# yharby/flac-raster

Hardware: AMD Instinct MI355X
Metric: raster MPixels/sec encoded at -c 5 + size ratio vs libFLAC, 1/2/4/8 GPU (higher is better)
Workload: dtype u16->i16 (int32 analysis, exact integer autocorrelation on i8 MFMA)

## Files before the change

### flac-raster_amd/csrc/fra_analyze_w.hip

```cpp
#include <type_traits>

#include "fra_device.h"

namespace fra {

namespace {

constexpr int kWChunks = kMaxBlock / kChunk;
constexpr int kWIters = kWChunks / 64;

struct WaveSmem {
  uint32_t sw[8 * kWChunks];
  double acf[3][9];
};
constexpr uint32_t kBufWords = 8 * kWChunks;

__device__ __forceinline__ int sdw(int t, int d) { return 8 * t + d; }
__device__ __forceinline__ int32_t wsample(const uint32_t* sw, int s) {
  const uint32_t v = sw[sdw(s >> 4, (s & 15) >> 1)];
  return (s & 1) ? hi16(v) : lo16(v);
}
__device__ __forceinline__ void wsync() {
  __builtin_amdgcn_wave_barrier();
  asm volatile("" ::: "memory");
}
constexpr int kWIterDw = 8 * 64;
constexpr int kWinW = 3;
__device__ __forceinline__ uint4 lds4(const uint32_t* p) { return *reinterpret_cast<const uint4*>(p); }
__device__ __forceinline__ void wread_d14(const uint32_t* sw, int lane, int j, uint32_t (&D)[14]) {
  const uint32_t* po = sw + 8 * lane + kWIterDw * j;
  const bool first = j == 0 && lane == 0;
  const uint32_t* pp = first ? po : po - 8;
  const uint4 p0 = lds4(pp), p1 = lds4(pp + 4), o0 = lds4(po), o1 = lds4(po + 4);
  D[0] = first ? 0u : p0.z; D[1] = first ? 0u : p0.w;
  D[2] = first ? 0u : p1.x; D[3] = first ? 0u : p1.y; D[4] = first ? 0u : p1.z; D[5] = first ? 0u : p1.w;
  D[6] = o0.x; D[7] = o0.y; D[8] = o0.z; D[9] = o0.w;
  D[10] = o1.x; D[11] = o1.y; D[12] = o1.z; D[13] = o1.w;
}
__device__ __forceinline__ void unpack28(const uint32_t (&D)[14], int32_t (&x)[28]) {
#pragma unroll
  for (int k = 0; k < 14; k++) {
    x[2 * k] = lo16(D[k]);
    x[2 * k + 1] = hi16(D[k]);
  }
}
__device__ __forceinline__ uint32_t group_sum32(uint32_t v, int ls) {
  if (ls > 0) v = up_add32<0>(v);
  if (ls > 1) v = up_add32<1>(v);
  if (ls > 2) v = up_add32<2>(v);
  if (ls > 3) v = up_add32<3>(v);
  if (ls > 4) v = up_add32<4>(v);
  if (ls > 5) v = up_add32<5>(v);
  return v;
}
__device__ __forceinline__ uint64_t group_sum64(uint64_t v, int ls) {
  if (ls > 0) v = up_add64<0>(v);
  if (ls > 1) v = up_add64<1>(v);
  if (ls > 2) v = up_add64<2>(v);
  if (ls > 3) v = up_add64<3>(v);
  if (ls > 4) v = up_add64<4>(v);
  if (ls > 5) v = up_add64<5>(v);
  return v;
}
__device__ __forceinline__ uint64_t group_sum_auto(uint64_t v, int ls) {
  if (__all(v < (1ull << (32 - ls)))) return group_sum32((uint32_t)v, ls);
  return group_sum64(v, ls);
}
__device__ __forceinline__ double rdlane_f64(double v, int l) {
  const uint64_t b = (uint64_t)__double_as_longlong(v);
  const uint32_t lo = (uint32_t)__builtin_amdgcn_readlane((int)(uint32_t)b, l);
  const uint32_t hi = (uint32_t)__builtin_amdgcn_readlane((int)(uint32_t)(b >> 32), l);
  return __longlong_as_double((long long)(((uint64_t)hi << 32) | lo));
}


__device__ __forceinline__ int32_t wround16(float x, float w) {
  return __float_as_int(__fadd_rn(__fmul_rn(x, w), 12582912.0f));
}

template <int MAXLAG>
__device__ inline int levinson_keep(const double (&ac)[MAXLAG + 1], int max_order, double& e, double (&lp)[MAXLAG],
                                    int lo) {
  double lpc[MAXLAG];
#pragma unroll
  for (int j = 0; j < MAXLAG; j++) { lpc[j] = 0.0; lp[j] = 0.0; }
  e = 0.0;
  double err = ac[0];
  int result = max_order;
  bool done = false;
#pragma unroll
  for (int i = 0; i < MAXLAG; i++) {
    if (!done && i < max_order) {
      double r = -ac[i + 1];
#pragma unroll
      for (int j = 0; j < i; j++) r = r - lpc[j] * ac[i - j];
      r = r / err;
      lpc[i] = r;
#pragma unroll
      for (int j = 0; j < (i >> 1); j++) {
        const double tmp = lpc[j];
        lpc[j] = lpc[j] + r * lpc[i - 1 - j];
        lpc[i - 1 - j] = lpc[i - 1 - j] + r * tmp;
      }
      if (i & 1) lpc[i >> 1] = lpc[i >> 1] + lpc[i >> 1] * r;
      err = err * (1.0 - r * r);
      const bool mine = lo == i + 1;
#pragma unroll
      for (int j = 0; j <= i; j++) lp[j] = mine ? -lpc[j] : lp[j];
      e = (mine || (i == 0 && lo == 0)) ? err : e;
      if (!(err > 0.0)) {
        result = (err == 0.0) ? i + 1 : i;
        done = true;
      }
    }
  }
  return result;
}

__device__ __forceinline__ void fixed_guess2_w(const uint32_t (&ps)[5], int P, int lane, int& g1, int& g2,
                                               uint64_t& t1, uint64_t& t2) {
  uint64_t T[5];
  bool small = true;
  uint32_t pv[5];
#pragma unroll
  for (int k = 0; k < 5; k++) {
    pv[k] = lane < (1 << P) ? ps[k] : 0u;
    small = small && pv[k] < (1u << 25);
  }
  if (__all(small)) {
#pragma unroll
    for (int k = 0; k < 5; k++) T[k] = wave_sum32(pv[k]);
  } else {
#pragma unroll
    for (int k = 0; k < 5; k++) {
      uint64_t v = pv[k];
      v = up_add64<0>(v); v = up_add64<1>(v); v = up_add64<2>(v);
      v = up_add64<3>(v); v = up_add64<4>(v); v = up_add64<5>(v);
      T[k] = ((uint64_t)(uint32_t)__builtin_amdgcn_readlane((int)(uint32_t)(v >> 32), 63) << 32) |
             (uint32_t)__builtin_amdgcn_readlane((int)(uint32_t)v, 63);
    }
  }
  int h1 = -1, h2 = -1;
  uint64_t b1 = 0, b2 = 0;
#pragma unroll
  for (int k = 0; k < 5; k++) {
    const bool lt1 = h1 < 0 || T[k] < b1;
    const bool lt2 = !lt1 && (h2 < 0 || T[k] < b2);
    b2 = lt1 ? b1 : (lt2 ? T[k] : b2);
    h2 = lt1 ? h1 : (lt2 ? k : h2);
    b1 = lt1 ? T[k] : b1;
    h1 = lt1 ? k : h1;
  }
  g1 = __builtin_amdgcn_readfirstlane(h1);
  g2 = __builtin_amdgcn_readfirstlane(h2);
  t1 = b1;
  t2 = b2;
}

#ifndef FRA_W_ARITH
#define FRA_W_ARITH 0
#endif
struct WNorm {
  double two_mn, range, rcp;
  uint32_t flip;
};
template <typename T>
__device__ __forceinline__ int32_t wnorm(uint32_t r, const WNorm& q) {
  const int32_t v = (int32_t)((r ^ q.flip) - q.flip);
  const double t = fma((double)v, 2.0, q.two_mn);
  const double q0 = t * q.rcp;
  const double rr = fma(-q0, q.range, t);
  double u = fma(rr, q.rcp, q0);
  u = u - 1.0;
  u = u * 32767.0;
  return (int32_t)u;
}
template <typename T>
__device__ __forceinline__ void wload_lut(const void* base, const WaveDev& wd, int c,
                                          const int32_t* lut, uint32_t* sw, int lane, uint32_t& orv, uint32_t& anv,
                                          bool stamp, const WNorm& wn) {
  constexpr int V = 8 / (int)sizeof(T);
  constexpr int NV = kMaxBlock / 64 / V;
  constexpr uint32_t step = 64 * V;
  using VT = VecT<T, V>;
  const uint32_t w = wd.width;
  const char* b0 = (const char*)((const T*)base + wd.off0 + (int64_t)c * wd.band_stride);
  const uint32_t rsb = wd.row_stride * (uint32_t)sizeof(T);
  const uint32_t qs = step / w, rs = step - qs * w, rstep = qs * rsb;
  uint32_t col = wd.col0 + (uint32_t)lane * V;
  uint32_t roff = 0;
  if (col >= w) {
    const uint32_t q = col / w;
    col -= q * w;
    roff = q * rsb;
  }
  VT x[NV];
#pragma unroll
  for (int kv = 0; kv < NV; kv++) {
    x[kv] = *(const VT*)(b0 + (roff + col * (uint32_t)sizeof(T)));
    col += rs;
    roff += rstep;
    if (col >= w) { col -= w; roff += rsb; }
  }
  if (stamp) FRA_WSTAMP_WAIT(11)
  uint32_t orp = 0, anp = 0xFFFFFFFFu;
#pragma unroll
  for (int kv = 0; kv < NV; kv++) {
    int32_t g[V];
    const bool arith = FRA_W_ARITH == 1 || (FRA_W_ARITH == 2 && (kv & 1));
    const uint2 xw = __builtin_bit_cast(uint2, x[kv]);
#pragma unroll
    for (int e = 0; e < V; e++) {
      constexpr int EB = 8 * (int)sizeof(T);
      const uint32_t wsrc = e < V / 2 ? xw.x : xw.y;
      const uint32_t raw = (wsrc >> (EB * (e % (V / 2)))) & ((1u << EB) - 1u);
      uint32_t off = raw << 2;
      asm("" : "+v"(off));
      g[e] = arith ? wnorm<T>(raw, wn) : *(const int32_t*)((const char*)lut + off);
    }
    const int i = (lane + 64 * kv) * V;
#pragma unroll
    for (int h = 0; h < V / 4; h++) {
      const int s = i + 4 * h;
      const uint32_t p0 = __builtin_amdgcn_perm((uint32_t)g[4 * h + 1], (uint32_t)g[4 * h], 0x05040100u);
      const uint32_t p1 = __builtin_amdgcn_perm((uint32_t)g[4 * h + 3], (uint32_t)g[4 * h + 2], 0x05040100u);
      *reinterpret_cast<uint2*>(&sw[sdw(s >> 4, (s & 15) >> 1)]) = make_uint2(p0, p1);
      orp |= p0 | p1;
      anp &= p0 & p1;
    }
  }
  orv |= (orp | (orp >> 16)) & 0xFFFFu;
  anv &= anp & (anp >> 16);
  if (stamp) FRA_WSTAMP_WAIT(12)
}

#define FRA_DOT4(a, b, c, d, q, c0, c1, c2, c3)                   \
  "v_dot2_i32_i16 %[p0], %[x" #a "], %[q" #q "], " c0 "\n\t"      \
  "v_dot2_i32_i16 %[p1], %[x" #b "], %[q" #q "], " c1 "\n\t"      \
  "v_dot2_i32_i16 %[p2], %[x" #c "], %[q" #q "], " c2 "\n\t"      \
  "v_dot2_i32_i16 %[p3], %[x" #d "], %[q" #q "], " c3 "\n\t"
#define FRA_DOT4_FIRST(a, b, c, d, q) FRA_DOT4(a, b, c, d, q, "0", "0", "0", "0")
#define FRA_DOT4_NEXT(a, b, c, d, q) FRA_DOT4(a, b, c, d, q, "%[p0]", "%[p1]", "%[p2]", "%[p3]")
#define FRA_SHR4                              \
  "v_ashrrev_i32 %[p0], %[sh], %[p0]\n\t"     \
  "v_ashrrev_i32 %[p1], %[sh], %[p1]\n\t"     \
  "v_ashrrev_i32 %[p2], %[sh], %[p2]\n\t"     \
  "v_ashrrev_i32 %[p3], %[sh], %[p3]"
#define FRA_P4_OUT [p0] "=&v"(p[0]), [p1] "=&v"(p[1]), [p2] "=&v"(p[2]), [p3] "=&v"(p[3])
template <int NP>
__device__ __forceinline__ void pred4_w(const uint32_t (&D)[14], int b, const fra_short2 (&Q)[NP], int sh,
                                        int32_t (&p)[4]) {
  static_assert(NP >= 1 && NP <= 4, "orders 1-8");
  uint32_t X[2 * NP + 2];
#pragma unroll
  for (int k = 0; k < 2 * NP + 2; k++) X[k] = pair_at(D, b - 2 * NP + k);
  if constexpr (NP == 1) {
    asm(FRA_DOT4_FIRST(0, 1, 2, 3, 0) FRA_SHR4
        : FRA_P4_OUT
        : [sh] "s"(sh), [q0] "s"(Q[0]), [x0] "v"(X[0]), [x1] "v"(X[1]), [x2] "v"(X[2]), [x3] "v"(X[3]));
  } else if constexpr (NP == 2) {
    asm(FRA_DOT4_FIRST(2, 3, 4, 5, 0) FRA_DOT4_NEXT(0, 1, 2, 3, 1) FRA_SHR4
        : FRA_P4_OUT
        : [sh] "s"(sh), [q0] "s"(Q[0]), [q1] "s"(Q[1]), [x0] "v"(X[0]), [x1] "v"(X[1]), [x2] "v"(X[2]), [x3] "v"(X[3]),
          [x4] "v"(X[4]), [x5] "v"(X[5]));
  } else if constexpr (NP == 3) {
    asm(FRA_DOT4_FIRST(4, 5, 6, 7, 0) FRA_DOT4_NEXT(2, 3, 4, 5, 1) FRA_DOT4_NEXT(0, 1, 2, 3, 2) FRA_SHR4
        : FRA_P4_OUT
        : [sh] "s"(sh), [q0] "s"(Q[0]), [q1] "s"(Q[1]), [q2] "s"(Q[2]), [x0] "v"(X[0]), [x1] "v"(X[1]), [x2] "v"(X[2]),
          [x3] "v"(X[3]), [x4] "v"(X[4]), [x5] "v"(X[5]), [x6] "v"(X[6]), [x7] "v"(X[7]));
  } else {
    asm(FRA_DOT4_FIRST(6, 7, 8, 9, 0) FRA_DOT4_NEXT(4, 5, 6, 7, 1) FRA_DOT4_NEXT(2, 3, 4, 5, 2)
        FRA_DOT4_NEXT(0, 1, 2, 3, 3) FRA_SHR4
        : FRA_P4_OUT
        : [sh] "s"(sh), [q0] "s"(Q[0]), [q1] "s"(Q[1]), [q2] "s"(Q[2]), [q3] "s"(Q[3]), [x0] "v"(X[0]), [x1] "v"(X[1]),
          [x2] "v"(X[2]), [x3] "v"(X[3]), [x4] "v"(X[4]), [x5] "v"(X[5]), [x6] "v"(X[6]), [x7] "v"(X[7]), [x8] "v"(X[8]),
          [x9] "v"(X[9]));
  }
}
#undef FRA_P4_OUT
#undef FRA_SHR4
#undef FRA_DOT4_NEXT
#undef FRA_DOT4_FIRST
#undef FRA_DOT4

template <int O>
__device__ __forceinline__ uint32_t lpc_abs16_w(const uint32_t (&D)[14], const int32_t* q, int sh, bool head) {
  constexpr int NP = (O + 1) / 2;
  fra_short2 Q[NP];
  q_pairs_rev<NP>(q, Q);
  uint32_t acc = 0;
#pragma unroll
  for (int jb = 0; jb < kChunk; jb += 4) {
    int32_t p[4];
    pred4_w<NP>(D, 12 + jb, Q, sh, p);
#pragma unroll
    for (int i = 0; i < 4; i++) {
      const int jj = jb + i;
      const int32_t r = sample_at(D, 12 + jj) - p[i];
      const uint32_t rb = (uint32_t)r ^ kBias;
      acc = sad_acc(rb, (jj < O && head) ? rb : kBias, acc);
    }
  }
  return acc;
}

template <int O, bool K17>
__device__ __forceinline__ uint32_t lpc_abs16_pk(const uint32_t (&D)[14], const int32_t* q, int sh, bool head,
                                                 uint32_t (&pk)[kChunk / 2], uint32_t& um, uint32_t& hb) {
  constexpr int NP = (O + 1) / 2;
  fra_short2 Q[NP];
  q_pairs_rev<NP>(q, Q);
  uint32_t su = 0, ss = 0;
  uint32_t u[kChunk];
  hb = 0;
#pragma unroll
  for (int jb = 0; jb < kChunk; jb += 4) {
    int32_t p[4];
    pred4_w<NP>(D, 12 + jb, Q, sh, p);
#pragma unroll
    for (int i = 0; i < 4; i++) {
      const int jj = jb + i;
      const int32_t r = sample_at(D, 12 + jj) - p[i];
      uint32_t sg = (uint32_t)(r >> 31);
      asm("" : "+v"(sg));
      const bool warm = jj < O && head;
      u[jj] = warm ? 0u : (((uint32_t)r << 1) ^ sg);
      su += u[jj];
      ss += warm ? 0u : sg;
      um |= u[jj];
    }
  }
  const uint32_t acc = su - ss;
#pragma unroll
  for (int p = 0; p < kChunk / 2; p++) pk[p] = __builtin_amdgcn_perm(u[2 * p + 1], u[2 * p], 0x05040100u);
  if (K17 && __any(um > 0xFFFFu)) {
#pragma unroll
    for (int jj = 0; jj < kChunk; jj++) hb |= (u[jj] >> 16) << jj;
  }
  return acc;
}

}


template <int MAXLAG, int PCAP, bool K17>
#ifndef FRA_W_WAVES
#define FRA_W_WAVES 4
#endif
#ifndef FRA_W_ACF_ITERS
#define FRA_W_ACF_ITERS 4
#endif
#ifndef FRA_W_VGPR_FLOOR
#define FRA_W_VGPR_FLOOR 1
#endif
#ifndef FRA_W_WAVES_MAX
#define FRA_W_WAVES_MAX 8
#endif
__global__ void __launch_bounds__(64) __attribute__((amdgpu_waves_per_eu(FRA_W_WAVES, FRA_W_WAVES_MAX)))
k_analyze_w(JobArgs a, int src) {
  static_assert(MAXLAG == 8 && PCAP >= 4 && PCAP <= 6, "levels 3-6");
  __shared__ WaveSmem S;
  uint32_t* const sw = S.sw;
  const int lane = (int)threadIdx.x;
#if FRA_W_VGPR_FLOOR
  asm volatile("" ::: "v103");
#endif
  FRA_WSTAMP(0)
#ifndef FRA_W_XCD
#define FRA_W_XCD 1
#endif
  int bx = (int)blockIdx.x;
  if (FRA_W_XCD) {
    const int nx = (int)gridDim.x, n8 = nx & ~7;
    const int lin = bx + (int)blockIdx.y * nx;
    if ((nx & 7) == 0 && bx < n8) bx = (lin & 7) * (n8 >> 3) + (bx >> 3);
  }
  const int g = a.frame_base + bx;
  const int c = (int)blockIdx.y;
  const WaveDev wd = a.wave[g];
  if (c >= wd.nch) return;
  FRA_WSTAMP_WAIT(10)
  if (wd.n != kMaxBlock) return;
  constexpr int n = kMaxBlock;
  const int bps = wd.bps;
  const LevelCfg cfg = level_cfg(a.level);
  SfDesc* d = &a.sf[(size_t)g * a.cmax + c];
  uint32_t* const slot = a.tmp + ((size_t)g * a.cmax + c) * a.tmp_stride;
#ifdef FRA_WSTOP
  if (lane == 0) {
    d->type = 1; d->order = 0; d->wasted = 0; d->sbps = (uint8_t)bps; d->cval = 0; d->porder = 0;
    d->method = 0; d->precision = 0; d->shift = 0; d->bits = 8u + (uint32_t)n * (uint32_t)bps;
  }
#endif

  uint32_t orv = 0, anv = 0xFFFFu;
  const void* const raster = a.raster;
  const int32_t* const lut = a.lut + (int64_t)wd.stream * a.lut_stride;
  WNorm wn{};
  if (FRA_W_ARITH) {
    const NormParams np = norm_params(a.streams[wd.stream], a.norm[wd.stream]);
    wn.two_mn = -2.0 * np.mn;
    wn.range = np.range;
    wn.rcp = np.rcp;
    wn.flip = src == ST_I16 ? 0x8000u : (src == ST_I8 ? 0x80u : 0u);
  }
  auto load_samples = [&](uint32_t& ov, uint32_t& an, bool first) {
    if (src == ST_U8 || src == ST_I8) wload_lut<uint8_t>(raster, wd, c, lut, sw, lane, ov, an, first, wn);
    else wload_lut<uint16_t>(raster, wd, c, lut, sw, lane, ov, an, first, wn);
  };
  load_samples(orv, anv, true);
  orv = wave_or32(orv);
  wsync();
  FRA_WSTAMP(1)
  anv = ~wave_or32(~anv) & 0xFFFFu;
  FRA_WSTOP_AT(1, orv ^ (anv << 16) ^ sw[lane] ^ sw[2047 - lane])

  if (anv == orv) {
    const int32_t vmin = lo16(orv);
    if (lane == 0) {
      d->type = 0; d->order = 0; d->wasted = 0; d->sbps = (uint8_t)bps; d->cval = vmin;
      d->bits = 8u + (uint32_t)bps; d->porder = 0; d->method = 0; d->precision = 0; d->shift = 0;
      const uint64_t v = (uint64_t)(uint32_t)vmin & ((1ull << bps) - 1);
      const uint64_t blob = v << (64 - 8 - bps);
      slot[0] = (uint32_t)(blob >> 32);
      slot[1] = (uint32_t)blob;
    }
    return;
  }
  const int w = __builtin_ctz(orv);
  const int sbps = bps - w;
  auto shift_wasted = [&]() {
    for (int k = lane; k < (int)kBufWords; k += 64) {
      const uint32_t v = sw[k];
      const uint32_t lo = (uint32_t)(lo16(v) >> w) & 0xFFFFu, hi = (uint32_t)(hi16(v) >> w);
      sw[k] = lo | (hi << 16);
    }
  };
  if (w) shift_wasted();
  wsync();
  const uint32_t hdr = 8u + (uint32_t)w;
  const uint32_t verb = hdr + (uint32_t)n * (uint32_t)sbps;
  constexpr int P = PCAP;
  constexpr int gsl = 8 - P;
  const int prec = qlp_precision(bps, n);
  const int lmax = cfg.max_lpc;

  constexpr int npl = 6 - gsl;
  const int pj = lane >> npl;
  const int psrc = ((lane & ((1 << npl) - 1)) << gsl) | ((1 << gsl) - 1);
  uint32_t pfix[5] = {0, 0, 0, 0, 0};
  for (int j = 0; j < kWIters; j += 2) {
    const int t = 64 * j + lane;
    const bool head = t == 0;
    uint32_t D[14];
    wread_d14(sw, lane, j, D);
    int32_t x[28];
    unpack28(D, x);
    uint32_t v[28];
#pragma unroll
    for (int jx = 8; jx < 28; jx++) v[jx] = (uint32_t)x[jx] ^ kBias;
#pragma unroll
    for (int k = 0; k <= 4; k++) {
      if (k > 1) {
#pragma unroll
        for (int jx = 12 + kChunk - 1; jx >= 7 + k; jx--) v[jx] = xad_bias(v[jx - 1], v[jx]);
      }
      uint32_t s32 = 0;
#pragma unroll
      for (int jj = 0; jj < kChunk; jj++) {
        const uint32_t ab = v[12 + jj];
        const uint32_t bb = k == 0 ? kBias : ((jj < k && head) ? ab : v[11 + jj]);
        s32 = sad_acc(ab, bb, s32);
      }
      const uint32_t gs = bperm32(group_sum32(s32, gsl), psrc);
      pfix[k] = pj == j ? 2u * gs : pfix[k];
    }
  }
  FRA_WSTAMP(2)
  FRA_WSTOP_AT(2, pfix[0] ^ pfix[1] ^ pfix[2] ^ pfix[3] ^ pfix[4])

  uint32_t west = 0xFFFFFFFFu;
  int wm = 99, wtype = 2, wo = 0, wsh = 0, wps = 0;
  uint32_t wk = 0;
  auto offer = [&](uint32_t est, int m, int type, int o, int sh, int ps, uint32_t kreg) {
    if (est < west || (est == west && m < wm)) {
      west = est; wm = m; wtype = type; wo = o; wsh = sh; wps = ps; wk = kreg;
    }
  };

  int g1, g2;
  uint64_t gt1, gt2;
  fixed_guess2_w(pfix, P, lane, g1, g2, gt1, gt2);
  uint32_t pf1 = 0, pf2 = 0;
#pragma unroll
  for (int k = 0; k < 5; k++) {
    pf1 = k == g1 ? pfix[k] : pf1;
    pf2 = k == g2 ? pfix[k] : pf2;
  }
  {
    const int kmax = g1 > g2 ? g1 : g2;
#pragma unroll 1
    for (int j = 1; j < kWIters; j += 2) {
      uint32_t D[14];
      wread_d14(sw, lane, j, D);
      int32_t x[28];
      unpack28(D, x);
      uint32_t v[28];
#pragma unroll
      for (int jx = 8; jx < 28; jx++) v[jx] = (uint32_t)x[jx] ^ kBias;
      uint32_t s1 = 0, s2 = 0;
#pragma unroll
      for (int k = 0; k <= 4; k++) {
        if (k > kmax) break;
        if (k > 1) {
#pragma unroll
          for (int jx = 12 + kChunk - 1; jx >= 7 + k; jx--) v[jx] = xad_bias(v[jx - 1], v[jx]);
        }
        if (k == g1 || k == g2) {
          uint32_t s32 = 0;
#pragma unroll
          for (int jj = 0; jj < kChunk; jj++) s32 = sad_acc(v[12 + jj], k == 0 ? kBias : v[11 + jj], s32);
          if (k == g1) s1 = s32;
          else s2 = s32;
        }
      }
      const uint32_t gs1 = bperm32(group_sum32(s1, gsl), psrc), gs2 = bperm32(group_sum32(s2, gsl), psrc);
      pf1 = pj == j ? 2u * gs1 : pf1;
      pf2 = pj == j ? 2u * gs2 : pf2;
    }
    gt1 = (uint64_t)wave_sum32(pf1);
    gt2 = (uint64_t)wave_sum32(pf2);
  }
#if defined(FRA_WPAD) && FRA_WPAD > 0
  {
    uint32_t p0 = lane, p1 = lane + 1, p2 = lane + 2, p3 = lane + 3;
#pragma unroll
    for (int k = 0; k < FRA_WPAD / 4; k++) {
      asm volatile("v_add_u32 %0, %0, %1" : "+v"(p0) : "v"(p1));
      asm volatile("v_add_u32 %0, %0, %1" : "+v"(p1) : "v"(p2));
      asm volatile("v_add_u32 %0, %0, %1" : "+v"(p2) : "v"(p3));
      asm volatile("v_add_u32 %0, %0, %1" : "+v"(p3) : "v"(p0));
    }
    asm volatile("" ::"v"(p0 ^ p1 ^ p2 ^ p3));
  }
#endif
  FRA_WSTAMP(3)
  FRA_WSTOP_AT(3, pf1 ^ pf2 ^ (uint32_t)(g1 * 8 + g2))
  int nlpc = 0;
  uint32_t mv = 0;
  if constexpr (MAXLAG > 0) {
    if (cfg.nsub > 0 && lmax > 0) {
      nlpc = a.nwin;
      const int nwin = a.nwin;
      constexpr int NL = MAXLAG + 1;
      double acl[NL];
      for (int wi = 0; wi < nwin; wi++) {
        const int32_t* wr = a.wrange + 2 * ((size_t)wd.win * a.nwin + wi);
        const int32_t* wp = a.wplat + 2 * ((size_t)wd.win * a.nwin + wi);
        const int lo = wr[0], hi = wr[1], plo = wp[0], phi = wp[1];
        const float* win = a.win + ((size_t)wd.win * a.nwin + wi) * a.blocksize;
        const int ri = lane & 15, g4 = lane >> 4;
        i32x4 c0h = {0, 0, 0, 0}, c0m = c0h, c0l = c0h, c1h = c0h, c1m = c0h, c1l = c0h;
        int32_t ysh = 0, ysl = 0, yfirst = 0;
        const int16_t* const sh16 = reinterpret_cast<const int16_t*>(sw);
        for (int blk = 0; blk < kWIters; blk++) {
          const int b0 = 1024 * blk;
          int sb = b0 + 256 * g4 + ri;
          asm volatile("" : "+v"(sb));
          const int16_t* const sp = sh16 + sb;
          const float* const wp = win + sb;
          const int kind = (!(lo < b0 + 1024 && hi > b0) || blk >= FRA_W_ACF_ITERS) ? 0
                           : (b0 >= plo && b0 + 1024 <= phi) ? 1 : 2;
          uint32_t H[5], L[5];
#pragma unroll
          for (int hf = 0; hf < 2; hf++) {
            int32_t y[8];
            if (kind == 0) {
#pragma unroll
              for (int e = 0; e < 8; e++) y[e] = 0;
            } else if (kind == 1) {
#pragma unroll
              for (int e = 0; e < 8; e++) y[e] = sp[16 * (8 * hf + e)];
            } else {
              float wc[8];
#pragma unroll
              for (int e = 0; e < 8; e++) wc[e] = wp[16 * (8 * hf + e)];
#pragma unroll
              for (int e = 0; e < 8; e++) y[e] = wround16((float)sp[16 * (8 * hf + e)], wc[e]);
            }
            if (blk == 0 && hf == 0) yfirst = lo16((uint32_t)y[0]);
#pragma unroll
            for (int dd = 0; dd < 2; dd++) {
              const uint32_t p01 = __builtin_amdgcn_perm((uint32_t)y[4 * dd + 1], (uint32_t)y[4 * dd], 0x05010400u);
              const uint32_t p23 = __builtin_amdgcn_perm((uint32_t)y[4 * dd + 3], (uint32_t)y[4 * dd + 2], 0x05010400u);
              L[2 * hf + dd] = __builtin_amdgcn_perm(p23, p01, 0x05040100u) ^ 0x80808080u;
              H[2 * hf + dd] = __builtin_amdgcn_perm(p23, p01, 0x07060302u);
              ysh = __builtin_amdgcn_sdot4((int)H[2 * hf + dd], 0x01010101, ysh, false);
              ysl = __builtin_amdgcn_sdot4((int)L[2 * hf + dd], 0x01010101, ysl, false);
            }
            if (hf == 0) asm volatile("" ::: "memory");
          }
          int32_t y16;
          {
            const bool in = blk < kWIters - 1 || g4 < 3;
            const float x16 = in ? (float)sp[256] : 0.0f;
            y16 = wround16(x16, in ? wp[256] : 0.0f);
          }
          H[4] = (uint32_t)y16 >> 8;
          L[4] = (uint32_t)y16 ^ 0x80u;
          const i32x4 xh = {(int)H[0], (int)H[1], (int)H[2], (int)H[3]};
          const i32x4 xl = {(int)L[0], (int)L[1], (int)L[2], (int)L[3]};
          const i32x4 sh = {(int)__builtin_amdgcn_alignbyte(H[1], H[0], 1), (int)__builtin_amdgcn_alignbyte(H[2], H[1], 1),
                            (int)__builtin_amdgcn_alignbyte(H[3], H[2], 1), (int)__builtin_amdgcn_alignbyte(H[4], H[3], 1)};
          const i32x4 sl = {(int)__builtin_amdgcn_alignbyte(L[1], L[0], 1), (int)__builtin_amdgcn_alignbyte(L[2], L[1], 1),
                            (int)__builtin_amdgcn_alignbyte(L[3], L[2], 1), (int)__builtin_amdgcn_alignbyte(L[4], L[3], 1)};
          c0h = __builtin_amdgcn_mfma_i32_16x16x64_i8(xh, xh, c0h, 0, 0, 0);
          c0m = __builtin_amdgcn_mfma_i32_16x16x64_i8(xh, xl, c0m, 0, 0, 0);
          c0m = __builtin_amdgcn_mfma_i32_16x16x64_i8(xl, xh, c0m, 0, 0, 0);
          c0l = __builtin_amdgcn_mfma_i32_16x16x64_i8(xl, xl, c0l, 0, 0, 0);
          c1h = __builtin_amdgcn_mfma_i32_16x16x64_i8(xh, sh, c1h, 0, 0, 0);
          c1m = __builtin_amdgcn_mfma_i32_16x16x64_i8(xh, sl, c1m, 0, 0, 0);
          c1m = __builtin_amdgcn_mfma_i32_16x16x64_i8(xl, sh, c1m, 0, 0, 0);
          c1l = __builtin_amdgcn_mfma_i32_16x16x64_i8(xl, sl, c1l, 0, 0, 0);
        }
        double mq = 0.0;
#pragma unroll
        for (int q = 0; q < 4; q++) {
          const int dd = ri - 4 * g4 - q;
          const bool in0 = dd >= 0;
          const double v = fma((double)(in0 ? c0h[q] : c1h[q]), 65536.0,
                               fma((double)(in0 ? c0m[q] : c1m[q]), 256.0, (double)(in0 ? c0l[q] : c1l[q])));
          mq = mq + __shfl(v, 16 * g4 + ((ri + 4 * g4 + q) & 15), 64);
        }
        mq = mq + __shfl_xor(mq, 16, 64);
        mq = mq + __shfl_xor(mq, 32, 64);
        const int32_t ytot = (int32_t)wave_sum32((uint32_t)(256 * ysh + ysl)) + 128 * kMaxBlock;
        int32_t pre = 0;
#pragma unroll
        for (int m = 0; m < MAXLAG; m++) {
          const int32_t vm = __builtin_amdgcn_readlane(yfirst, m);
          pre += ri > m ? vm : 0;
        }
        const double rl = mq + (256.0 * (double)ytot - 128.0 * (double)pre - 67108864.0);
        if (lane < NL) S.acf[wi][lane] = rl;
      }
      wsync();
      {
        const int gw = min(lane >> 4, nwin - 1);
#pragma unroll
        for (int l = 0; l < NL; l++) acl[l] = S.acf[gw][l];
      }
      FRA_WSTAMP(4)
#ifdef FRA_WSTOP
      {
        uint64_t kx = 0;
#pragma unroll
        for (int l = 0; l < NL; l++) kx ^= (uint64_t)__double_as_longlong(acl[l]);
        FRA_WSTOP_AT(4, kx ^ (kx >> 32))
      }
#endif
      const int gw = lane >> 4, lo = lane & 15;
      const bool gon = gw < nwin;
      double lpo[MAXLAG], e = 0.0;
      int nord = 0;
      if (gon && acl[0] != 0.0) nord = levinson_keep<MAXLAG>(acl, lmax, e, lpo, lo);
      const bool on = nord > 0 && lo >= 1 && lo <= nord;
      const uint64_t key = on ? (uint64_t)__double_as_longlong(order_bits(e, n, lo, prec + sbps)) : ~0ull;
      uint64_t rk = min(key, dpp64_old<DPP_SHR1, 0xF>(key, ~0ull));
      rk = min(rk, dpp64_old<DPP_SHR2, 0xF>(rk, ~0ull));
      rk = min(rk, dpp64_old<DPP_SHR4, 0xF>(rk, ~0ull));
      rk = min(rk, dpp64_old<DPP_SHR8, 0xF>(rk, ~0ull));
      const uint64_t kmin = __shfl(rk, (lane & 48) | 15, 64);
      const uint64_t bal = __ballot(on && key == kmin);
      const uint32_t rowbits = (uint32_t)(bal >> (16 * gw)) & 0xFFFFu;
      int32_t q[MAXLAG];
#pragma unroll
      for (int jx = 0; jx < MAXLAG; jx++) q[jx] = 0;
      bool ok = false;
      int qsh = 0;
      if (on) ok = quantize<MAXLAG>(lpo, lo, prec, q, qsh);
      const int o_l = nord > 0 ? (int)__builtin_ctz(rowbits | 0x10000u) : 0;
      const int dwi = lane < 24 ? lane >> 3 : (lane - 24) & 3;
      const int ow = (int)bperm32((uint32_t)o_l, 16 * dwi);
      const int L = 16 * dwi + ow;
      const uint32_t info = (uint32_t)qsh | ((o_l > 0 && ok) ? (uint32_t)o_l << 8 : 0u);
      const uint32_t vinfo = bperm32(info, L);
#pragma unroll
      for (int jx = 0; jx < 8; jx++) {
        const uint32_t vq = bperm32((uint32_t)q[jx], L);
        mv = (lane & 7) == jx ? vq : mv;
      }
      mv = lane >= 24 ? vinfo : mv;
      mv = (lane < 24 ? dwi : lane - 24) < nwin && lane < 27 ? mv : 0u;
    }
  }
  FRA_WSTAMP(5)
#ifdef FRA_WSTOP
  {
    const uint32_t kx = wave_or32(mv ^ (uint32_t)lane);
    FRA_WSTOP_AT(5, kx)
  }
#endif

  const uint32_t okm = (uint32_t)(__ballot(lane >= 24 && lane < 24 + kWinW && (mv >> 8) != 0) >> 24);
#ifndef FRA_W_KEEP
#define FRA_W_KEEP 0
#endif
  const int keep_wi = okm ? (FRA_W_KEEP ? 31 - __clz((int)okm) : __builtin_ctz(okm)) : -1;
  bool kept_fit = false;
  uint64_t hk = 0;
  bool hk_any = false;
  uint32_t w4[4] = {0, 0, 0, 0};
  uint64_t lpcT = ~0ull;
#pragma unroll 1
  for (int ci = 0; ci < nlpc + 2; ci++) {
    int m, o, sh = 0, type = 2;
    int32_t qm[8] = {0, 0, 0, 0, 0, 0, 0, 0};
    uint64_t psum = 0;
    if (ci >= nlpc) {
      m = o = ci == nlpc ? g1 : g2;
      if (o < 0 || (lpcT != ~0ull && (ci == nlpc ? gt1 : gt2) >= lpcT)) continue;
      psum = ci == nlpc ? pf1 : pf2;
    } else {
      const int wi = (ci + keep_wi + 1) % nlpc;
      if (!((okm >> wi) & 1u)) continue;
      const uint32_t inf = (uint32_t)__builtin_amdgcn_readlane((int)mv, 24 + wi);
      o = (int)(inf >> 8);
      m = 5 + wi;
      type = 3;
      sh = (int)(inf & 0xFFu);
#pragma unroll
      for (int jx = 0; jx < 8; jx++) qm[jx] = __builtin_amdgcn_readlane((int)mv, 8 * wi + jx);
      if (wi == keep_wi) {
        uint32_t um = 0, carry[6] = {0, 0, 0, 0, 0, 0};
        auto keep_iter = [&](const int j, auto headc) {
          constexpr bool kHead = decltype(headc)::value;
          const bool head = kHead && lane == 0;
          uint32_t* const po = sw + 8 * lane + kWIterDw * j;
          uint32_t D[14];
          wread_d14(sw, lane, j, D);
          if (j > 0) {
#pragma unroll
            for (int k = 0; k < 6; k++) D[k] = lane == 0 ? carry[k] : D[k];
          }
#pragma unroll
          for (int k = 0; k < 6; k++) carry[k] = (uint32_t)__builtin_amdgcn_readlane((int)D[8 + k], 63);
          if (j == 0) {
#pragma unroll
            for (int k = 0; k < 4; k++) w4[k] = (uint32_t)__builtin_amdgcn_readlane((int)D[6 + k], 0);
          }
          uint32_t acc = 0, pk[kChunk / 2], hb = 0;
          switch (o) {
#define FRA_CASE(O_) \
  case O_: acc = lpc_abs16_pk<O_, K17>(D, qm, sh, head, pk, um, hb); break;
            FRA_CASE(1) FRA_CASE(2) FRA_CASE(3) FRA_CASE(4) FRA_CASE(5) FRA_CASE(6) FRA_CASE(7) FRA_CASE(8)
#undef FRA_CASE
          }
          wsync();
#pragma unroll
          for (int p = 0; p < kChunk / 4; p++) *reinterpret_cast<uint2*>(po + 2 * p) = make_uint2(pk[2 * p], pk[2 * p + 1]);
          hk |= (uint64_t)hb << (16 * j);
          const uint64_t gs = bperm64(group_sum_auto((uint64_t)acc, gsl), psrc);
          psum = pj == j ? gs : psum;
        };
        keep_iter(0, std::true_type{});
#pragma unroll 1
        for (int j = 1; j < kWIters; j++) keep_iter(j, std::false_type{});
        const bool need17 = __any(um > 0xFFFFu) && !__any(um > 0x1FFFFu);
        if (need17 && lane == 0 && a.cnt17) atomicAdd(a.cnt17, 1u);
        if constexpr (K17) {
          kept_fit = !__any(um > 0x1FFFFu);
          hk_any = __any(hk != 0);
        } else {
          kept_fit = !__any(um > 0xFFFFu);
        }
      } else {
#pragma unroll 1
        for (int j = 0; j < kWIters; j++) {
          const int t = 64 * j + lane;
          const bool head = t == 0;
          uint32_t D[14];
          wread_d14(sw, lane, j, D);
          uint32_t acc = 0;
          switch (o) {
#define FRA_CASE(O_) \
  case O_: acc = lpc_abs16_w<O_>(D, qm, sh, head); break;
            FRA_CASE(1) FRA_CASE(2) FRA_CASE(3) FRA_CASE(4) FRA_CASE(5) FRA_CASE(6) FRA_CASE(7) FRA_CASE(8)
#undef FRA_CASE
          }
          const uint64_t gs = bperm64(group_sum_auto(2ull * acc, gsl), psrc);
          psum = pj == j ? gs : psum;
        }
      }
      uint64_t tv = psum;
      tv = up_add64<0>(tv); tv = up_add64<1>(tv); tv = up_add64<2>(tv);
      tv = up_add64<3>(tv); tv = up_add64<4>(tv); tv = up_add64<5>(tv);
      const uint64_t T = ((uint64_t)(uint32_t)__builtin_amdgcn_readlane((int)(uint32_t)(tv >> 32), 63) << 32) |
                         (uint32_t)__builtin_amdgcn_readlane((int)(uint32_t)tv, 63);
      lpcT = T < lpcT ? T : lpcT;
    }
    constexpr int pm = P;
    uint64_t best;
    int bp;
    uint32_t kreg;
    porder_search_reg(psum, P, pm, n, o, lane, best, bp, kreg);
    const uint64_t est = hdr + (uint64_t)o * sbps + (type == 3 ? 9 + (uint64_t)o * prec : 0) + best;
    offer((uint32_t)est, m, type, o, sh, bp, kreg);
  }

  FRA_WSTAMP(6)
  FRA_WSTOP_AT(6, west ^ (uint32_t)wm ^ (uint32_t)wps)
  const int type = wtype, o = wo, sh = wsh, ps = wps;
  int32_t wq[8];
#pragma unroll
  for (int jq = 0; jq < 8; jq++) wq[jq] = type == 3 ? __builtin_amdgcn_readlane((int)mv, 8 * (wm - 5) + jq) : 0;
  const bool kept_w = type == 3 && wm == 5 + keep_wi && kept_fit;
  FRA_WSTAMP_VAL(9, kept_w ? 0 : (type != 3 ? 3 : (wm != 5 + keep_wi ? 4 : 5)))
  auto reload = [&]() {
    wsync();
    uint32_t ov = 0, an = 0;
    load_samples(ov, an, false);
    wsync();
    if (w) shift_wasted();
    wsync();
  };
  const int pz = n >> ps;
  const int tl = 8 - ps;
  const int ls = tl < 6 ? tl : 6;
  const int npp = 1 << ps;
  auto tail = [&](auto kept_tag) {
    constexpr bool kept = decltype(kept_tag)::value;
    int32_t warm = 0;
    if (kept) {
      const uint32_t wv2 = lane >= 6 ? w4[3] : lane >= 4 ? w4[2] : lane >= 2 ? w4[1] : w4[0];
      warm = lane < o ? ((lane & 1) ? hi16(wv2) : lo16(wv2)) : 0;
    } else if (lane < o) {
      warm = wsample(sw, lane);
    }
    fra_short2 Q[4];
    q_pairs_rev<4>(wq, Q);
    auto residuals = [&](int j, uint32_t (&un)[kChunk], uint32_t (&cy)[6]) {
      const int t = 64 * j + lane;
      if (kept) {
        const uint32_t* po = sw + 8 * lane + kWIterDw * j;
#pragma unroll
        for (int p = 0; p < kChunk / 4; p++) {
          const uint2 v = *reinterpret_cast<const uint2*>(po + 2 * p);
          un[4 * p] = v.x & 0xFFFFu;
          un[4 * p + 1] = v.x >> 16;
          un[4 * p + 2] = v.y & 0xFFFFu;
          un[4 * p + 3] = v.y >> 16;
        }
        if (hk_any) {
          const uint32_t h = (uint32_t)(hk >> (16 * j));
#pragma unroll
          for (int jj = 0; jj < kChunk; jj++) un[jj] |= ((h >> jj) & 1u) << 16;
        }
        return;
      }
      uint32_t D[14];
      wread_d14(sw, lane, j, D);
      if (j > 0) {
#pragma unroll
        for (int k = 0; k < 6; k++) D[k] = lane == 0 ? cy[k] : D[k];
      }
#pragma unroll
      for (int k = 0; k < 6; k++) cy[k] = (uint32_t)__builtin_amdgcn_readlane((int)D[8 + k], 63);
      if (type == 3) {
#pragma unroll
        for (int jb = 0; jb < kChunk; jb += 4) {
          int32_t p[4];
          pred4_w<4>(D, 12 + jb, Q, sh, p);
#pragma unroll
          for (int i = 0; i < 4; i++) un[jb + i] = zz32(sample_at(D, 12 + jb + i) - p[i]);
        }
      } else {
        int32_t x[28];
        unpack28(D, x);
#pragma unroll
        for (int k = 1; k <= 4; k++) {
          if (k <= o) {
#pragma unroll
            for (int jx = 12 + kChunk - 1; jx >= 8 + k; jx--) x[jx] = x[jx] - x[jx - 1];
          }
        }
#pragma unroll
        for (int jj = 0; jj < kChunk; jj++) un[jj] = zz32(x[12 + jj]);
      }
#pragma unroll
      for (int jj = 0; jj < 12; jj++)
        if (t == 0 && jj < o) un[jj] = 0u;
    };
    uint32_t kc[kWIters];
    uint32_t fk[kWIters][3];
    uint32_t k0r[kWIters];
    uint32_t bitsl = 0;
    bool bigl = false;
    uint64_t E[3] = {0, 0, 0};
    uint32_t cyx[6] = {0, 0, 0, 0, 0, 0};
#pragma unroll
    for (int j = 0; j < kWIters; j++) {
      const int t = 64 * j + lane;
      const int pidx = t >> tl;
      const int k0 = __shfl((int)wk, pidx & 63, 64);
      const int km = k0 > 0 ? k0 - 1 : 0;
      uint32_t f0 = 0, f1 = 0, f2 = 0;
      if constexpr (kept) {
        const uint32_t* po = sw + 8 * lane + kWIterDw * j;
        typedef unsigned short u16x2 __attribute__((ext_vector_type(2)));
        auto sh = [](int k) -> u16x2 {
          const unsigned short c = (unsigned short)(k < 15 ? k : 15);
          return u16x2{c, c};
        };
        auto wt = [](int k) -> u16x2 {
          const unsigned short c = k < 16 ? 1 : 0;
          return u16x2{c, c};
        };
        const u16x2 sm = sh(km), s0 = sh(k0), s1 = sh(k0 + 1), mm = wt(km), m0 = wt(k0), m1 = wt(k0 + 1);
        if (hk_any) {
          const uint32_t c = (uint32_t)__builtin_popcount((uint32_t)(hk >> (16 * j)) & 0xFFFFu);
          f0 = km <= 16 ? c << (16 - km) : 0u;
          f1 = k0 <= 16 ? c << (16 - k0) : 0u;
          f2 = k0 + 1 <= 16 ? c << (15 - k0) : 0u;
        }
#pragma unroll
        for (int p = 0; p < kChunk / 4; p++) {
          const uint2 v = *reinterpret_cast<const uint2*>(po + 2 * p);
          const u16x2 w0 = __builtin_bit_cast(u16x2, v.x), w1 = __builtin_bit_cast(u16x2, v.y);
          f0 = __builtin_amdgcn_udot2(w0 >> sm, mm, f0, false);
          f0 = __builtin_amdgcn_udot2(w1 >> sm, mm, f0, false);
          f1 = __builtin_amdgcn_udot2(w0 >> s0, m0, f1, false);
          f1 = __builtin_amdgcn_udot2(w1 >> s0, m0, f1, false);
          f2 = __builtin_amdgcn_udot2(w0 >> s1, m1, f2, false);
          f2 = __builtin_amdgcn_udot2(w1 >> s1, m1, f2, false);
        }
      } else {
        uint32_t un[kChunk];
        residuals(j, un, cyx);
#pragma unroll
        for (int jj = 0; jj < kChunk; jj++) {
          f0 += un[jj] >> km;
          f1 += un[jj] >> k0;
          f2 += un[jj] >> (k0 + 1);
        }
      }
      fk[j][0] = f0;
      fk[j][1] = f1;
      fk[j][2] = f2;
      k0r[j] = (uint32_t)k0;
      uint64_t v0, v1, v2;
      if (kept || __all(f0 <= (0xFFFFFFFFu >> ls))) {
        v0 = group_sum32(f0, ls); v1 = group_sum32(f1, ls); v2 = group_sum32(f2, ls);
      } else {
        v0 = group_sum64(f0, ls); v1 = group_sum64(f1, ls); v2 = group_sum64(f2, ls);
      }
      if (tl <= 6) {
        const uint32_t cnt = (uint32_t)(pz - (pidx == 0 ? o : 0));
        const uint64_t ev[3] = {v0, v1, v2};
        uint64_t best = 0;
        int bk = 0;
        bool first = true;
#pragma unroll
        for (int dk = -1; dk <= 1; dk++) {
          const int kk = k0 + dk;
          const uint64_t e = (uint64_t)(cnt * (uint32_t)(kk + 1)) + ev[dk + 1];
          const bool take = kk >= 0 && kk <= 30 && (first || e < best);
          best = take ? e : best;
          bk = take ? kk : bk;
          first = first && !(kk >= 0 && kk <= 30);
// ... 51 lines not shown
      return false;
    }
    if (!kept && verbatim) {
      if (lane == 0) {
        d->type = 1; d->order = 0; d->wasted = (uint8_t)w; d->sbps = (uint8_t)sbps; d->cval = 0; d->porder = 0;
        d->method = 0; d->precision = 0; d->shift = 0; d->bits = verb;
      }
      const uint32_t nwv = (verb + 31) >> 5;
      const uint64_t hv = ((uint64_t)(2u | (w ? 1u : 0u)) << 56) | (w ? (1ull << (63 - (8 + w - 1))) : 0ull);
      for (uint32_t jw = lane; jw < nwv; jw += 64) {
        const int64_t wb = 32 * (int64_t)jw;
        uint32_t word = jw == 0 ? (uint32_t)(hv >> 32) : (jw == 1 ? (uint32_t)hv : 0u);
        const int s0 = wb > (int64_t)hdr ? (int)((wb - (int64_t)hdr) / sbps) : 0;
        for (int s = s0; s < n && (int64_t)hdr + (int64_t)s * sbps < wb + 32; s++) {
          const int64_t rel = (int64_t)hdr + (int64_t)s * sbps - wb;
          const int sft = 32 - (int)rel - sbps;
          const uint64_t v = (uint64_t)((uint32_t)wsample(sw, s) & smask);
          word |= sft >= 0 ? (uint32_t)(v << sft) : (uint32_t)(v >> -sft);
        }
        slot[jw] = word;
      }
      return true;
    }
    const uint32_t fbits = (uint32_t)exact;
    const uint32_t nw = (fbits + 31) >> 5;
    const int pb = big ? 5 : 4;
    const uint32_t pos = hdr + (uint32_t)o * sbps + (type == 3 ? 9u + (uint32_t)o * prec : 0u);
    uint32_t excl[kWIters];
    uint32_t B[kWIters + 1];
    B[0] = pos + 6;
#pragma unroll
    for (int j = 0; j < kWIters; j++) {
      const int t = 64 * j + lane;
      const uint32_t kcur = kc[j], k0 = k0r[j];
      const uint32_t f = kcur + 1 == k0 ? fk[j][0] : kcur == k0 ? fk[j][1] : fk[j][2];
      const bool pstart = ((t << 4) & (pz - 1)) == 0;
      const uint32_t tot = f + (uint32_t)(kChunk - (t == 0 ? o : 0)) * (kcur + 1u) + (pstart ? (uint32_t)pb : 0u);
      const uint32_t sc = wave_incl_scan32(tot);
      excl[j] = sc - tot;
      B[j + 1] = B[j] + (uint32_t)__builtin_amdgcn_readlane((int)sc, 63);
    }
    bool inlds = nw + 1 <= kBufWords;
#pragma unroll
    for (int j = 0; j + 1 < kWIters; j++) inlds = inlds && (B[j + 1] - 1) / 32 + 2 <= (uint32_t)sdw(64 * (j + 1), 0);
    if (kept && !inlds) {
      FRA_WSTAMP_VAL(9, 7)
      return false;
    }
    if (lane < kMaxLpc) {
      int32_t cv = 0;
#pragma unroll
      for (int jq = 0; jq < 8; jq++) cv = lane == jq ? wq[jq] : cv;
      d->coef[lane] = type == 3 ? cv : 0;
    }
    if (lane == 0) {
      d->wasted = (uint8_t)w; d->sbps = (uint8_t)sbps; d->cval = 0;
      d->type = (uint8_t)type; d->order = (uint8_t)o; d->porder = (uint8_t)ps; d->method = big ? 1 : 0;
      d->precision = (uint8_t)(type == 3 ? prec : 0); d->shift = (int8_t)sh; d->bits = (uint32_t)exact;
    }
    auto put_header = [&](uint32_t* buf) {
      if (lane == 0) {
        lds_put(buf, 0, (uint32_t)((type == 3 ? 31 + o : 8 + o) << 1) | (w ? 1u : 0u), 8);
        if (w) lds_put(buf, 8 + (uint32_t)(w - 1), 1u, 1);
      }
      if (lane < o) lds_put(buf, hdr + (uint32_t)lane * sbps, (uint32_t)warm & smask, sbps);
      const uint32_t ph = hdr + (uint32_t)o * sbps;
      if (type == 3 && lane == 0) {
        lds_put(buf, ph, (uint32_t)(prec - 1), 4);
        lds_put(buf, ph + 4, (uint32_t)sh & 31u, 5);
      }
      if (type == 3 && lane < o) {
        int32_t cv = 0;
#pragma unroll
        for (int jq = 0; jq < 8; jq++) cv = lane == jq ? wq[jq] : cv;
        lds_put(buf, ph + 9 + (uint32_t)lane * prec, (uint32_t)cv & ((1u << prec) - 1u), prec);
      }
      if (lane == 0) lds_put(buf, pos, ((uint32_t)(big ? 1 : 0) << 4) | (uint32_t)ps, 6);
    };
    auto put_codes = [&](uint32_t* buf, int j, const uint32_t (&un)[kChunk]) {
      const int t = 64 * j + lane;
      const bool head = t == 0;
      const uint32_t kcur = kc[j];
      const bool pstart = ((t << 4) & (pz - 1)) == 0;
      uint32_t p = B[j] + excl[j];
      if (pstart) { lds_put(buf, p, kcur, pb); p += (uint32_t)pb; }
      const uint32_t sal = 31u - kcur;
#pragma unroll
      for (int jj = 0; jj < kChunk; jj++) {
        const bool skip = jj < 12 && head && jj < o;
        const uint32_t Pp = p + (un[jj] >> kcur);
        lds_put_al(buf, Pp, skip ? 0u : ((un[jj] << sal) | 0x80000000u));
        p = skip ? p : Pp + 1u + kcur;
      }
    };
    uint32_t cye[6] = {0, 0, 0, 0, 0, 0};
    if (kept || inlds) {
      uint32_t* const buf = sw;
      uint32_t Z = 0;
#pragma unroll
      for (int j = 0; j < kWIters; j++) {
        uint32_t un[kChunk];
        residuals(j, un, cye);
        wsync();
        const uint32_t Zend = j == kWIters - 1 ? nw + 1 : (B[j + 1] - 1) / 32 + 2;
        for (uint32_t jw = Z + lane; jw < Zend; jw += 64) buf[jw] = 0u;
        Z = Zend > Z ? Zend : Z;
        wsync();
        if (j == 0) put_header(buf);
        put_codes(buf, j, un);
      }
      wsync();
      for (uint32_t jw = lane; jw < nw; jw += 64) slot[jw] = buf[jw];
      FRA_WSTAMP(8)
    } else {
      for (uint32_t jw = lane; jw <= nw; jw += 64) slot[jw] = 0u;
      __threadfence();
      put_header(slot);
#pragma unroll 1
      for (int j = 0; j < kWIters; j++) {
        uint32_t un[kChunk];
        residuals(j, un, cye);
        put_codes(slot, j, un);
      }
    }
    return true;
  };
  if (!kept_w || !tail(std::true_type{})) {
    if (keep_wi >= 0) reload();
    tail(std::false_type{});
  }
}

#ifdef FRA_STAMPS
}
extern "C" __attribute__((visibility("default"))) int fra_diag_wstamps(void* host, unsigned long long bytes) {
  if (!host) {
    void* d = nullptr;
    if (hipGetSymbolAddress(&d, HIP_SYMBOL(fra::g_fra_wstamps)) != hipSuccess) return -1;
    return hipMemset(d, 0, sizeof(fra::g_fra_wstamps)) == hipSuccess ? 0 : -1;
  }
  const size_t nb = bytes < sizeof(fra::g_fra_wstamps) ? bytes : sizeof(fra::g_fra_wstamps);
  return hipMemcpyFromSymbol(host, HIP_SYMBOL(fra::g_fra_wstamps), nb, 0, hipMemcpyDeviceToHost) == hipSuccess ? 0 : -1;
}
namespace fra {
#endif

hipError_t launch_analyze_w(int src, int level, const JobArgs& a, int cw, hipStream_t s) {
  const bool k17 = a.k17 != 0;
  if (a.frame_count <= 0) return hipSuccess;
  const dim3 grid((unsigned)a.frame_count, (unsigned)cw);
  const LevelCfg cfg = level_cfg(level);
  if (cfg.nsub == 0 || cfg.max_lpc > 8) return hipErrorInvalidValue;
  if (!a.wave) return hipErrorInvalidValue;
  switch (cfg.max_porder) {
    case 4: k17 ? k_analyze_w<8, 4, true><<<grid, 64, 0, s>>>(a, src) : k_analyze_w<8, 4, false><<<grid, 64, 0, s>>>(a, src); break;
    case 5: k17 ? k_analyze_w<8, 5, true><<<grid, 64, 0, s>>>(a, src) : k_analyze_w<8, 5, false><<<grid, 64, 0, s>>>(a, src); break;
    default: k17 ? k_analyze_w<8, 6, true><<<grid, 64, 0, s>>>(a, src) : k_analyze_w<8, 6, false><<<grid, 64, 0, s>>>(a, src); break;
  }
  return hipGetLastError();
}

}
```

Before: 99990.

## Specialize wave analyzer for single window, early-stop Levinson, simplify row loads

Adds a compile-time window count tied to the partition cap so levels below 6 use a single apodization window. This replaces permute-based coefficient gathering with readlane and drops the non-kept window re-estimation loop. Levinson recursion now stops at each lane's own order and broadcasts the final order from lane 15, cutting redundant double-precision work. Sample loads take a simpler per-row addressing path when the width and start column are aligned to the load step. The launcher now rejects window counts that do not match the level, which ties correctness to the host configuration.

```diff
diff --git a/flac-raster_amd/csrc/fra_analyze_w.hip b/flac-raster_amd/csrc/fra_analyze_w.hip
--- a/flac-raster_amd/csrc/fra_analyze_w.hip
+++ b/flac-raster_amd/csrc/fra_analyze_w.hip
@@ -26,6 +26,7 @@
 }
 constexpr int kWIterDw = 8 * 64;
 constexpr int kWinW = 3;
+constexpr int wave_nwin(int pcap) { return pcap == 6 ? kWinW : 1; }
 __device__ __forceinline__ uint4 lds4(const uint32_t* p) { return *reinterpret_cast<const uint4*>(p); }
 __device__ __forceinline__ void wread_d14(const uint32_t* sw, int lane, int j, uint32_t (&D)[14]) {
   const uint32_t* po = sw + 8 * lane + kWIterDw * j;
@@ -78,6 +79,9 @@
   return __float_as_int(__fadd_rn(__fmul_rn(x, w), 12582912.0f));
 }
 
+#ifndef FRA_W_LEV_STOP
+#define FRA_W_LEV_STOP 1
+#endif
 template <int MAXLAG>
 __device__ inline int levinson_keep(const double (&ac)[MAXLAG + 1], int max_order, double& e, double (&lp)[MAXLAG],
                                     int lo) {
@@ -88,9 +92,10 @@
   double err = ac[0];
   int result = max_order;
   bool done = false;
+  const int last = FRA_W_LEV_STOP ? (lo > 1 ? lo : 1) : MAXLAG;
 #pragma unroll
   for (int i = 0; i < MAXLAG; i++) {
-    if (!done && i < max_order) {
+    if (!done && i < max_order && i < last) {
       double r = -ac[i + 1];
 #pragma unroll
       for (int j = 0; j < i; j++) r = r - lpc[j] * ac[i - j];
@@ -104,15 +109,22 @@
       }
       if (i & 1) lpc[i >> 1] = lpc[i >> 1] + lpc[i >> 1] * r;
       err = err * (1.0 - r * r);
-      const bool mine = lo == i + 1;
-#pragma unroll
-      for (int j = 0; j <= i; j++) lp[j] = mine ? -lpc[j] : lp[j];
-      e = (mine || (i == 0 && lo == 0)) ? err : e;
+      if (!FRA_W_LEV_STOP) {
+        const bool mine = lo == i + 1;
+#pragma unroll
+        for (int j = 0; j <= i; j++) lp[j] = mine ? -lpc[j] : lp[j];
+        e = (mine || (i == 0 && lo == 0)) ? err : e;
+      }
       if (!(err > 0.0)) {
         result = (err == 0.0) ? i + 1 : i;
         done = true;
       }
     }
+  }
+  if (FRA_W_LEV_STOP) {
+#pragma unroll
+    for (int j = 0; j < MAXLAG; j++) lp[j] = -lpc[j];
+    e = err;
   }
   return result;
 }
@@ -159,6 +171,9 @@
 
 #ifndef FRA_W_ARITH
 #define FRA_W_ARITH 0
+#endif
+#ifndef FRA_W_SROW
+#define FRA_W_SROW 1
 #endif
 struct WNorm {
   double two_mn, range, rcp;
@@ -187,20 +202,31 @@
   const char* b0 = (const char*)((const T*)base + wd.off0 + (int64_t)c * wd.band_stride);
   const uint32_t rsb = wd.row_stride * (uint32_t)sizeof(T);
   const uint32_t qs = step / w, rs = step - qs * w, rstep = qs * rsb;
-  uint32_t col = wd.col0 + (uint32_t)lane * V;
-  uint32_t roff = 0;
-  if (col >= w) {
-    const uint32_t q = col / w;
-    col -= q * w;
-    roff = q * rsb;
-  }
   VT x[NV];
-#pragma unroll
-  for (int kv = 0; kv < NV; kv++) {
-    x[kv] = *(const VT*)(b0 + (roff + col * (uint32_t)sizeof(T)));
-    col += rs;
-    roff += rstep;
-    if (col >= w) { col -= w; roff += rsb; }
+  if (FRA_W_SROW && w % step == 0 && wd.col0 % step == 0) {
+    const uint32_t lb = (uint32_t)lane * 8u;
+    uint32_t scol = wd.col0, sroff = 0;
+#pragma unroll
+    for (int kv = 0; kv < NV; kv++) {
+      x[kv] = *(const VT*)(b0 + (sroff + scol * (uint32_t)sizeof(T)) + lb);
+      scol += step;
+      if (scol >= w) { scol = 0; sroff += rsb; }
+    }
+  } else {
+    uint32_t col = wd.col0 + (uint32_t)lane * V;
+    uint32_t roff = 0;
+    if (col >= w) {
+      const uint32_t q = col / w;
+      col -= q * w;
+      roff = q * rsb;
+    }
+#pragma unroll
+    for (int kv = 0; kv < NV; kv++) {
+      x[kv] = *(const VT*)(b0 + (roff + col * (uint32_t)sizeof(T)));
+      col += rs;
+      roff += rstep;
+      if (col >= w) { col -= w; roff += rsb; }
+    }
   }
   if (stamp) FRA_WSTAMP_WAIT(11)
   uint32_t orp = 0, anp = 0xFFFFFFFFu;
@@ -359,6 +385,7 @@
 __global__ void __launch_bounds__(64) __attribute__((amdgpu_waves_per_eu(FRA_W_WAVES, FRA_W_WAVES_MAX)))
 k_analyze_w(JobArgs a, int src) {
   static_assert(MAXLAG == 8 && PCAP >= 4 && PCAP <= 6, "levels 3-6");
+  constexpr int NWIN = wave_nwin(PCAP);
   __shared__ WaveSmem S;
   uint32_t* const sw = S.sw;
   const int lane = (int)threadIdx.x;
@@ -550,15 +577,15 @@
   uint32_t mv = 0;
   if constexpr (MAXLAG > 0) {
     if (cfg.nsub > 0 && lmax > 0) {
-      nlpc = a.nwin;
-      const int nwin = a.nwin;
+      const int nwin = NWIN == 1 ? 1 : a.nwin;
+      nlpc = nwin;
       constexpr int NL = MAXLAG + 1;
       double acl[NL];
       for (int wi = 0; wi < nwin; wi++) {
-        const int32_t* wr = a.wrange + 2 * ((size_t)wd.win * a.nwin + wi);
-        const int32_t* wp = a.wplat + 2 * ((size_t)wd.win * a.nwin + wi);
+        const int32_t* wr = a.wrange + 2 * ((size_t)wd.win * nwin + wi);
+        const int32_t* wp = a.wplat + 2 * ((size_t)wd.win * nwin + wi);
         const int lo = wr[0], hi = wr[1], plo = wp[0], phi = wp[1];
-        const float* win = a.win + ((size_t)wd.win * a.nwin + wi) * a.blocksize;
+        const float* win = a.win + ((size_t)wd.win * nwin + wi) * a.blocksize;
         const int ri = lane & 15, g4 = lane >> 4;
         i32x4 c0h = {0, 0, 0, 0}, c0m = c0h, c0l = c0h, c1h = c0h, c1m = c0h, c1l = c0h;
         int32_t ysh = 0, ysl = 0, yfirst = 0;
@@ -664,6 +691,10 @@
       double lpo[MAXLAG], e = 0.0;
       int nord = 0;
       if (gon && acl[0] != 0.0) nord = levinson_keep<MAXLAG>(acl, lmax, e, lpo, lo);
+      if (FRA_W_LEV_STOP) {
+        if constexpr (NWIN == 1) nord = gon ? __builtin_amdgcn_readlane(nord, 15) : 0;
+        else nord = __shfl(nord, lane | 15, 64);
+      }
       const bool on = nord > 0 && lo >= 1 && lo <= nord;
       const uint64_t key = on ? (uint64_t)__double_as_longlong(order_bits(e, n, lo, prec + sbps)) : ~0ull;
       uint64_t rk = min(key, dpp64_old<DPP_SHR1, 0xF>(key, ~0ull));
@@ -680,18 +711,29 @@
       int qsh = 0;
       if (on) ok = quantize<MAXLAG>(lpo, lo, prec, q, qsh);
       const int o_l = nord > 0 ? (int)__builtin_ctz(rowbits | 0x10000u) : 0;
-      const int dwi = lane < 24 ? lane >> 3 : (lane - 24) & 3;
-      const int ow = (int)bperm32((uint32_t)o_l, 16 * dwi);
-      const int L = 16 * dwi + ow;
       const uint32_t info = (uint32_t)qsh | ((o_l > 0 && ok) ? (uint32_t)o_l << 8 : 0u);
-      const uint32_t vinfo = bperm32(info, L);
-#pragma unroll
-      for (int jx = 0; jx < 8; jx++) {
-        const uint32_t vq = bperm32((uint32_t)q[jx], L);
-        mv = (lane & 7) == jx ? vq : mv;
-      }
-      mv = lane >= 24 ? vinfo : mv;
-      mv = (lane < 24 ? dwi : lane - 24) < nwin && lane < 27 ? mv : 0u;
+      if constexpr (NWIN == 1) {
+        const int L = __builtin_amdgcn_readfirstlane(o_l);
+        const uint32_t vinfo = (uint32_t)__builtin_amdgcn_readlane((int)info, L);
+#pragma unroll
+        for (int jx = 0; jx < 8; jx++) {
+          const uint32_t vq = (uint32_t)__builtin_amdgcn_readlane(q[jx], L);
+          mv = lane == jx ? vq : mv;
+        }
+        mv = lane == 24 ? vinfo : mv;
+      } else {
+        const int dwi = lane < 24 ? lane >> 3 : (lane - 24) & 3;
+        const int ow = (int)bperm32((uint32_t)o_l, 16 * dwi);
+        const int L = 16 * dwi + ow;
+        const uint32_t vinfo = bperm32(info, L);
+#pragma unroll
+        for (int jx = 0; jx < 8; jx++) {
+          const uint32_t vq = bperm32((uint32_t)q[jx], L);
+          mv = (lane & 7) == jx ? vq : mv;
+        }
+        mv = lane >= 24 ? vinfo : mv;
+        mv = (lane < 24 ? dwi : lane - 24) < nwin && lane < 27 ? mv : 0u;
+      }
     }
   }
   FRA_WSTAMP(5)
@@ -702,11 +744,12 @@
   }
 #endif
 
-  const uint32_t okm = (uint32_t)(__ballot(lane >= 24 && lane < 24 + kWinW && (mv >> 8) != 0) >> 24);
+  const uint32_t okm = NWIN == 1 ? (((uint32_t)__builtin_amdgcn_readlane((int)mv, 24) >> 8) != 0 ? 1u : 0u)
+                                 : (uint32_t)(__ballot(lane >= 24 && lane < 24 + kWinW && (mv >> 8) != 0) >> 24);
 #ifndef FRA_W_KEEP
 #define FRA_W_KEEP 0
 #endif
-  const int keep_wi = okm ? (FRA_W_KEEP ? 31 - __clz((int)okm) : __builtin_ctz(okm)) : -1;
+  const int keep_wi = okm ? (NWIN == 1 ? 0 : FRA_W_KEEP ? 31 - __clz((int)okm) : __builtin_ctz(okm)) : -1;
   bool kept_fit = false;
   uint64_t hk = 0;
   bool hk_any = false;
@@ -722,8 +765,9 @@
       if (o < 0 || (lpcT != ~0ull && (ci == nlpc ? gt1 : gt2) >= lpcT)) continue;
       psum = ci == nlpc ? pf1 : pf2;
     } else {
-      const int wi = (ci + keep_wi + 1) % nlpc;
+      const int wi = NWIN == 1 ? 0 : (ci + keep_wi + 1) % nlpc;
       if (!((okm >> wi) & 1u)) continue;
+      const bool keep_pass = NWIN == 1 || wi == keep_wi;
       const uint32_t inf = (uint32_t)__builtin_amdgcn_readlane((int)mv, 24 + wi);
       o = (int)(inf >> 8);
       m = 5 + wi;
@@ -731,7 +775,7 @@
       sh = (int)(inf & 0xFFu);
 #pragma unroll
       for (int jx = 0; jx < 8; jx++) qm[jx] = __builtin_amdgcn_readlane((int)mv, 8 * wi + jx);
-      if (wi == keep_wi) {
+      if (keep_pass) {
         uint32_t um = 0, carry[6] = {0, 0, 0, 0, 0, 0};
         auto keep_iter = [&](const int j, auto headc) {
           constexpr bool kHead = decltype(headc)::value;
@@ -774,7 +818,7 @@
         } else {
           kept_fit = !__any(um > 0xFFFFu);
         }
-      } else {
+      } else if constexpr (NWIN > 1) {
 #pragma unroll 1
         for (int j = 0; j < kWIters; j++) {
           const int t = 64 * j + lane;
@@ -813,8 +857,9 @@
   const int type = wtype, o = wo, sh = wsh, ps = wps;
   int32_t wq[8];
 #pragma unroll
-  for (int jq = 0; jq < 8; jq++) wq[jq] = type == 3 ? __builtin_amdgcn_readlane((int)mv, 8 * (wm - 5) + jq) : 0;
-  const bool kept_w = type == 3 && wm == 5 + keep_wi && kept_fit;
+  for (int jq = 0; jq < 8; jq++)
+    wq[jq] = type == 3 ? __builtin_amdgcn_readlane((int)mv, (NWIN == 1 ? 0 : 8 * (wm - 5)) + jq) : 0;
+  const bool kept_w = type == 3 && (NWIN == 1 || wm == 5 + keep_wi) && kept_fit;
   FRA_WSTAMP_VAL(9, kept_w ? 0 : (type != 3 ? 3 : (wm != 5 + keep_wi ? 4 : 5)))
   auto reload = [&]() {
     wsync();
@@ -1172,6 +1217,7 @@
   const LevelCfg cfg = level_cfg(level);
   if (cfg.nsub == 0 || cfg.max_lpc > 8) return hipErrorInvalidValue;
   if (!a.wave) return hipErrorInvalidValue;
+  if (a.nwin != wave_nwin(cfg.max_porder >= 6 ? 6 : cfg.max_porder)) return hipErrorInvalidValue;
   switch (cfg.max_porder) {
     case 4: k17 ? k_analyze_w<8, 4, true><<<grid, 64, 0, s>>>(a, src) : k_analyze_w<8, 4, false><<<grid, 64, 0, s>>>(a, src); break;
     case 5: k17 ? k_analyze_w<8, 5, true><<<grid, 64, 0, s>>>(a, src) : k_analyze_w<8, 5, false><<<grid, 64, 0, s>>>(a, src); break;
```

Result: faster. 102,600, median of 6 (+2.6%).
